# lszmer/metaquest-3d-reconstruction

Hardware: AMD Instinct MI355X
Metric: depth frames/sec integrated + mesh-extract ms, 512³ @ 5 mm; HBM GB/s vs peak (higher is better)
Workload: dtype f32

## Files before the change

### metaquest-3d-reconstruction_amd/csrc/meshfilter.hip

```cpp
#include <hipcub/hipcub.hpp>

#include <algorithm>
#include <cmath>
#include <limits>
#include <map>
#include <mutex>
#include <unordered_map>
#include <vector>

#include "device_block.hpp"
#include "mqr_common.hpp"

namespace mqr {
namespace mf {

__global__ void k_iota(int32_t* a, int64_t n) {
    const int64_t i = (int64_t)blockIdx.x * blockDim.x + threadIdx.x;
    if (i < n) a[i] = (int32_t)i;
}

__global__ void k_edge_keys(const int32_t* __restrict__ tri, int64_t nt, uint64_t* keys, int32_t* slot) {
    const int64_t i = (int64_t)blockIdx.x * blockDim.x + threadIdx.x;
    if (i >= 3 * nt) return;
    const int64_t t = i / 3;
    const int k = (int)(i % 3);
    const uint32_t a = (uint32_t)tri[3 * t + k], b = (uint32_t)tri[3 * t + (k + 1) % 3];
    keys[i] = a < b ? ((uint64_t)a << 32 | b) : ((uint64_t)b << 32 | a);
    slot[i] = (int32_t)i;
}

__device__ inline int32_t uf_find(int32_t* p, int32_t x) {
    while (true) {
        const int32_t px = p[x];
        if (px == x) return x;
        const int32_t gx = p[px];
        if (gx != px) p[x] = gx;
        x = gx;
    }
}

__global__ void k_union_edges(const uint64_t* __restrict__ keys, const int32_t* __restrict__ slot, int64_t m,
                              int32_t* parent) {
    const int64_t i = (int64_t)blockIdx.x * blockDim.x + threadIdx.x;
    if (i == 0 || i >= m || keys[i] != keys[i - 1]) return;
    int32_t a = slot[i - 1] / 3, b = slot[i] / 3;
    while (true) {
        a = uf_find(parent, a);
        b = uf_find(parent, b);
        if (a == b) return;
        if (a > b) {
            const int32_t t = a;
            a = b;
            b = t;
        }
        if (atomicCAS(&parent[b], b, a) == b) return;
    }
}

__global__ void k_roots(int32_t* parent, int64_t n, int32_t* count, int32_t* is_root) {
    const int64_t i = (int64_t)blockIdx.x * blockDim.x + threadIdx.x;
    const int lane = threadIdx.x & 63;
    int32_t r = -1;
    if (i < n) {
        r = uf_find(parent, (int32_t)i);
        is_root[i] = r == (int32_t)i;
    }
    bool todo = i < n;
    while (true) {
        const uint64_t pending = __ballot(todo);
        if (!pending) break;
        const int leader = __ffsll((unsigned long long)pending) - 1;
        const int32_t lr = __shfl(r, leader, 64);
        const bool same = todo && r == lr;
        const uint64_t peers = __ballot(same);
        if (lane == leader) atomicAdd(&count[lr], __popcll(peers));
        if (same) todo = false;
    }
}

__global__ void k_final_root(const int32_t* __restrict__ parent, int64_t n, int32_t* root) {
    const int64_t i = (int64_t)blockIdx.x * blockDim.x + threadIdx.x;
    if (i >= n) return;
    int32_t x = (int32_t)i;
    while (parent[x] != x) x = parent[x];
    root[i] = x;
}

__global__ void k_cluster_table(const int32_t* __restrict__ is_root, const int32_t* __restrict__ cid,
                                const int32_t* __restrict__ count, int64_t n, int32_t* ccount) {
    const int64_t i = (int64_t)blockIdx.x * blockDim.x + threadIdx.x;
    if (i < n && is_root[i]) ccount[cid[i]] = count[i];
}

__global__ void k_keep_by_cluster(const int32_t* __restrict__ root, const int32_t* __restrict__ cid,
                                  const uint8_t* __restrict__ keep_cluster, int64_t n, uint8_t* keep) {
    const int64_t i = (int64_t)blockIdx.x * blockDim.x + threadIdx.x;
    if (i < n) keep[i] = keep_cluster[cid[root[i]]];
}

__global__ void k_gather_tris(const int32_t* __restrict__ tri, const int32_t* __restrict__ sel, int64_t m,
                              int32_t* out) {
    const int64_t i = (int64_t)blockIdx.x * blockDim.x + threadIdx.x;
    if (i >= m) return;
    const int64_t s = sel[i];
    out[3 * i] = tri[3 * s];
    out[3 * i + 1] = tri[3 * s + 1];
    out[3 * i + 2] = tri[3 * s + 2];
}

__global__ void k_mark_vertices(const int32_t* __restrict__ tri, int64_t nt, int32_t* used) {
    const int64_t i = (int64_t)blockIdx.x * blockDim.x + threadIdx.x;
    if (i < 3 * nt) used[tri[i]] = 1;
}

__global__ void k_remap(int32_t* tri, int64_t nt, const int32_t* __restrict__ map) {
    const int64_t i = (int64_t)blockIdx.x * blockDim.x + threadIdx.x;
    if (i < 3 * nt) tri[i] = map[tri[i]];
}

__global__ void k_gather_vertices(const float* __restrict__ pos, const float* __restrict__ nrm,
                                  const int32_t* __restrict__ sel, int64_t m, float* pos_out, float* nrm_out) {
    const int64_t i = (int64_t)blockIdx.x * blockDim.x + threadIdx.x;
    if (i >= m) return;
    const int64_t s = sel[i];
    for (int a = 0; a < 3; ++a) {
        pos_out[3 * i + a] = pos[3 * s + a];
        if (nrm) nrm_out[3 * i + a] = nrm[3 * s + a];
    }
}

__global__ void k_not_degenerate(const int32_t* __restrict__ tri, int64_t nt, uint8_t* keep) {
    const int64_t i = (int64_t)blockIdx.x * blockDim.x + threadIdx.x;
    if (i >= nt) return;
    const int32_t a = tri[3 * i], b = tri[3 * i + 1], c = tri[3 * i + 2];
    keep[i] = a != b && b != c && c != a;
}

__device__ inline void canon(const int32_t* t, uint32_t& k0, uint32_t& k1, uint32_t& k2) {
    const uint32_t a = (uint32_t)t[0], b = (uint32_t)t[1], c = (uint32_t)t[2];
    if (a <= b) {
        if (a <= c) k0 = a, k1 = b, k2 = c;
        else k0 = c, k1 = a, k2 = b;
    } else {
        if (b <= c) k0 = b, k1 = c, k2 = a;
        else k0 = c, k1 = a, k2 = b;
    }
}

__global__ void k_tri_key_lo(const int32_t* __restrict__ tri, int64_t nt, uint32_t* k2, int32_t* idx) {
    const int64_t i = (int64_t)blockIdx.x * blockDim.x + threadIdx.x;
    if (i >= nt) return;
    uint32_t a, b, c;
    canon(tri + 3 * i, a, b, c);
    k2[i] = c;
    idx[i] = (int32_t)i;
}

__global__ void k_tri_key_hi(const int32_t* __restrict__ tri, const int32_t* __restrict__ idx, int64_t nt,
                             uint64_t* k01) {
    const int64_t i = (int64_t)blockIdx.x * blockDim.x + threadIdx.x;
    if (i >= nt) return;
    uint32_t a, b, c;
    canon(tri + 3 * (int64_t)idx[i], a, b, c);
    k01[i] = (uint64_t)a << 32 | b;
}

__global__ void k_first_of_run_tri(const int32_t* __restrict__ tri, const int32_t* __restrict__ idx, int64_t nt,
                                   uint8_t* keep) {
    const int64_t i = (int64_t)blockIdx.x * blockDim.x + threadIdx.x;
    if (i >= nt) return;
    uint32_t a, b, c;
    canon(tri + 3 * (int64_t)idx[i], a, b, c);
    bool first = i == 0;
    if (!first) {
        uint32_t pa, pb, pc;
        canon(tri + 3 * (int64_t)idx[i - 1], pa, pb, pc);
        first = a != pa || b != pb || c != pc;
    }
    keep[idx[i]] = first;
}

__device__ inline uint32_t coord_bits(float f) {
    const uint32_t u = __float_as_uint(f);
    return (u & 0x7fffffffu) == 0 ? 0u : u;
}
__device__ inline bool has_nan(const float* p) { return p[0] != p[0] || p[1] != p[1] || p[2] != p[2]; }

__global__ void k_vtx_key_lo(const float* __restrict__ pos, int64_t nv, uint32_t* kz, int32_t* idx) {
    const int64_t i = (int64_t)blockIdx.x * blockDim.x + threadIdx.x;
    if (i >= nv) return;
    kz[i] = coord_bits(pos[3 * i + 2]);
    idx[i] = (int32_t)i;
}

__global__ void k_vtx_key_hi(const float* __restrict__ pos, const int32_t* __restrict__ idx, int64_t nv,
                             uint64_t* kxy) {
    const int64_t i = (int64_t)blockIdx.x * blockDim.x + threadIdx.x;
    if (i >= nv) return;
    const float* p = pos + 3 * (int64_t)idx[i];
    kxy[i] = (uint64_t)coord_bits(p[0]) << 32 | coord_bits(p[1]);
}

__global__ void k_vtx_heads(const float* __restrict__ pos, const int32_t* __restrict__ idx, int64_t nv,
                            int32_t* head) {
    const int64_t i = (int64_t)blockIdx.x * blockDim.x + threadIdx.x;
    if (i >= nv) return;
    const float* p = pos + 3 * (int64_t)idx[i];
    bool first = i == 0 || has_nan(p);
    if (!first) {
        const float* q = pos + 3 * (int64_t)idx[i - 1];
        first = has_nan(q) || coord_bits(p[0]) != coord_bits(q[0]) || coord_bits(p[1]) != coord_bits(q[1]) ||
                coord_bits(p[2]) != coord_bits(q[2]);
    }
    head[i] = first ? (int32_t)i : 0;
}

__global__ void k_vtx_rep(const int32_t* __restrict__ idx, const int32_t* __restrict__ start, int64_t nv,
                          int32_t* rep, int32_t* keepv) {
    const int64_t i = (int64_t)blockIdx.x * blockDim.x + threadIdx.x;
    if (i >= nv) return;
    const int32_t v = idx[i], r = idx[start[i]];
    rep[v] = r;
    keepv[v] = r == v;
}

__global__ void k_vtx_map(const int32_t* __restrict__ rep, const int32_t* __restrict__ newidx, int64_t nv,
                          int32_t* map) {
    const int64_t i = (int64_t)blockIdx.x * blockDim.x + threadIdx.x;
    if (i < nv) map[i] = newidx[rep[i]];
}

__global__ void k_areas(const float* __restrict__ pos, const int32_t* __restrict__ tri, int64_t nt, double* area) {
    const int64_t i = (int64_t)blockIdx.x * blockDim.x + threadIdx.x;
    if (i >= nt) return;
    const float* p0 = pos + 3 * (int64_t)tri[3 * i];
    const float* p1 = pos + 3 * (int64_t)tri[3 * i + 1];
    const float* p2 = pos + 3 * (int64_t)tri[3 * i + 2];
    const double x0 = (double)p0[0] - p1[0], x1 = (double)p0[1] - p1[1], x2 = (double)p0[2] - p1[2];
    const double y0 = (double)p0[0] - p2[0], y1 = (double)p0[1] - p2[1], y2 = (double)p0[2] - p2[2];
    const double c0 = x1 * y2 - x2 * y1, c1 = x2 * y0 - x0 * y2, c2 = x0 * y1 - x1 * y0;
    area[i] = 0.5 * sqrt((c0 * c0 + c1 * c1) + c2 * c2);
}

__global__ void k_nonmanifold_members(const uint64_t* __restrict__ keys, int64_t m, uint8_t* flag) {
    const int64_t i = (int64_t)blockIdx.x * blockDim.x + threadIdx.x;
    if (i >= m) return;
    const uint64_t k = keys[i];
    const bool p1 = i >= 1 && keys[i - 1] == k, p2 = i >= 2 && keys[i - 2] == k;
    const bool n1 = i + 1 < m && keys[i + 1] == k, n2 = i + 2 < m && keys[i + 2] == k;
    flag[i] = (p1 && p2) || (p1 && n1) || (n1 && n2);
}

__global__ void k_gather_members(const uint64_t* __restrict__ keys, const int32_t* __restrict__ slot,
                                 const double* __restrict__ area, const int32_t* __restrict__ mem, int64_t n,
                                 uint64_t* okey, int32_t* otri, double* oarea) {
    const int64_t i = (int64_t)blockIdx.x * blockDim.x + threadIdx.x;
    if (i >= n) return;
    const int32_t e = mem[i], t = slot[e] / 3;
    okey[i] = keys[e];
    otri[i] = t;
    oarea[i] = area[t];
}

__global__ void k_drop_tris(const int32_t* __restrict__ del, int64_t n, double* area) {
    const int64_t i = (int64_t)blockIdx.x * blockDim.x + threadIdx.x;
    if (i < n) area[del[i]] = -1.0;
}

__global__ void k_keep_positive(const double* __restrict__ area, int64_t nt, uint8_t* keep) {
    const int64_t i = (int64_t)blockIdx.x * blockDim.x + threadIdx.x;
    if (i < nt) keep[i] = area[i] > 0;
}

__global__ void k_gather_f64(const double* __restrict__ a, const int32_t* __restrict__ sel, int64_t m, double* out) {
    const int64_t i = (int64_t)blockIdx.x * blockDim.x + threadIdx.x;
    if (i < m) out[i] = a[sel[i]];
}

inline unsigned nb(int64_t n) { return (unsigned)std::max<int64_t>((n + 255) / 256, 1); }

struct Arena {
    GrowBuf buf;
    bool busy = false;
    hipStream_t s = nullptr;
};
static std::mutex g_arena_mu;
static Arena g_arena[kMaxDevices];

struct Ctx {
    hipStream_t s = nullptr;
    int device = 0;
    Arena* ar = nullptr;
    Arena priv;
    size_t top = 0;
    std::vector<std::pair<size_t, size_t>> stack;
    std::vector<void*> owned;

    int open(int dev, size_t want) {
        device = dev;
        {
            std::lock_guard<std::mutex> lk(g_arena_mu);
            if (dev >= 0 && dev < kMaxDevices && !g_arena[dev].busy) {
                ar = &g_arena[dev];
                ar->busy = true;
            }
        }
        if (!ar) ar = &priv;
        if (!ar->s && hipStreamCreateWithFlags(&ar->s, hipStreamNonBlocking) != hipSuccess) return 1;
        s = ar->s;
        return ar->buf.reserve(want, want) != hipSuccess;
    }
    template <class T>
    T* alloc(int64_t n) {
        const size_t bytes = al256(sizeof(T) * (size_t)std::max<int64_t>(n, 1));
        if (ar && top + bytes <= ar->buf.cap) {
            stack.emplace_back(top, bytes);
            void* p = ar->buf.as<char>() + top;
            top += bytes;
            return static_cast<T*>(p);
        }
        void* p = nullptr;
        if (hipMallocAsync(&p, bytes, s) != hipSuccess) return nullptr;
        owned.push_back(p);
        return static_cast<T*>(p);
    }
    void release(void* p) {
        char* base = ar ? ar->buf.as<char>() : nullptr;
        if (ar && p >= (void*)base && p < (void*)(base + ar->buf.cap)) {
            const size_t off = static_cast<char*>(p) - base;
            for (size_t i = stack.size(); i-- > 0;)
                if (stack[i].first == off) {
                    stack.erase(stack.begin() + (std::ptrdiff_t)i);
                    break;
                }
            top = stack.empty() ? 0 : stack.back().first + stack.back().second;
            return;
        }
        auto it = std::find(owned.begin(), owned.end(), p);
        if (it != owned.end()) {
            (void)hipFreeAsync(p, s);
            owned.erase(it);
        }
    }
    ~Ctx() {
        if (!s) return;
        for (void* p : owned) (void)hipFreeAsync(p, s);
        (void)hipStreamSynchronize(s);
        if (ar == &priv) {
            if (priv.buf.p) (void)hipFree(priv.buf.p);
            (void)hipStreamDestroy(priv.s);
        } else if (ar) {
            std::lock_guard<std::mutex> lk(g_arena_mu);
            ar->busy = false;
        }
    }
};

#define MF_ALLOC(var, T, n)                                                      \
    T* var = c.alloc<T>(n);                                                      \
    if (!var) {                                                                  \
        set_error("mesh filter: device allocation failed");                      \
        return 1;                                                                \
    }

template <class F>
static int select_flagged(Ctx& c, const F* flags, int64_t n, int32_t* out, int64_t* count) {
    hipcub::CountingInputIterator<int32_t> it(0);
    int32_t* d_num = c.alloc<int32_t>(1);
    size_t tb = 0;
    MQR_CHECK_HIP(hipcub::DeviceSelect::Flagged(nullptr, tb, it, flags, out, d_num, (int)n, c.s));
    void* tmp = c.alloc<char>((int64_t)tb + 16);
    if (!d_num || !tmp) {
        set_error("mesh filter: device allocation failed");
        return 1;
    }
    MQR_CHECK_HIP(hipcub::DeviceSelect::Flagged(tmp, tb, it, flags, out, d_num, (int)n, c.s));
    int32_t h = 0;
    MQR_CHECK_HIP(hipMemcpyAsync(&h, d_num, sizeof(int32_t), hipMemcpyDeviceToHost, c.s));
    MQR_CHECK_HIP(hipStreamSynchronize(c.s));
    c.release(tmp);
    c.release(d_num);
    *count = h;
    return 0;
}

static int exclusive_sum(Ctx& c, const int32_t* in, int32_t* out, int64_t n) {
    size_t tb = 0;
    MQR_CHECK_HIP(hipcub::DeviceScan::ExclusiveSum(nullptr, tb, in, out, (int)n, c.s));
    void* tmp = c.alloc<char>((int64_t)tb + 16);
    if (!tmp) {
        set_error("mesh filter: device allocation failed");
        return 1;
    }
    MQR_CHECK_HIP(hipcub::DeviceScan::ExclusiveSum(tmp, tb, in, out, (int)n, c.s));
    c.release(tmp);
    return 0;
}

template <class K>
static int sort_pairs(Ctx& c, const K* kin, K* kout, const int32_t* vin, int32_t* vout, int64_t n, int bits) {
    size_t tb = 0;
    MQR_CHECK_HIP(hipcub::DeviceRadixSort::SortPairs(nullptr, tb, kin, kout, vin, vout, (int)n, 0, bits, c.s));
    void* tmp = c.alloc<char>((int64_t)tb + 16);
    if (!tmp) {
        set_error("mesh filter: device allocation failed");
        return 1;
    }
    MQR_CHECK_HIP(hipcub::DeviceRadixSort::SortPairs(tmp, tb, kin, kout, vin, vout, (int)n, 0, bits, c.s));
    c.release(tmp);
    return 0;
}

struct Mesh {
    float* pos = nullptr;
    float* nrm = nullptr;
    int32_t* tri = nullptr;
    int64_t nv = 0, nt = 0;
};

static int keep_triangles(Ctx& c, Mesh& m, const uint8_t* keep) {
    MF_ALLOC(sel, int32_t, m.nt);
    int64_t k = 0;
    if (select_flagged(c, keep, m.nt, sel, &k)) return 1;
    if (k == m.nt) {
        c.release(sel);
        return 0;
    }
    MF_ALLOC(tri2, int32_t, 3 * k);
    if (k) hipLaunchKernelGGL(k_gather_tris, dim3(nb(k)), dim3(256), 0, c.s, m.tri, sel, k, tri2);
    MQR_CHECK_HIP(hipGetLastError());
    c.release(sel);
    c.release(m.tri);
    m.tri = tri2;
    m.nt = k;
    return 0;
}

static int keep_vertices(Ctx& c, Mesh& m, const int32_t* keepv, const int32_t* map) {
    MF_ALLOC(sel, int32_t, m.nv);
    int64_t k = 0;
    if (select_flagged(c, keepv, m.nv, sel, &k)) return 1;
    if (m.nt) hipLaunchKernelGGL(k_remap, dim3(nb(3 * m.nt)), dim3(256), 0, c.s, m.tri, m.nt, map);
    MQR_CHECK_HIP(hipGetLastError());
    if (k != m.nv) {
        MF_ALLOC(pos2, float, 3 * k);
        float* nrm2 = nullptr;
        if (m.nrm) {
            nrm2 = c.alloc<float>(3 * k);
            if (!nrm2) {
                set_error("mesh filter: device allocation failed");
                return 1;
            }
        }
        if (k) hipLaunchKernelGGL(k_gather_vertices, dim3(nb(k)), dim3(256), 0, c.s, m.pos, m.nrm, sel, k, pos2, nrm2);
        MQR_CHECK_HIP(hipGetLastError());
        c.release(m.pos);
        if (m.nrm) c.release(m.nrm);
        m.pos = pos2;
        m.nrm = nrm2;
        m.nv = k;
    }
    c.release(sel);
    return 0;
}

static int remove_unreferenced_vertices(Ctx& c, Mesh& m) {
    MF_ALLOC(used, int32_t, m.nv);
    MF_ALLOC(newidx, int32_t, m.nv);
    MQR_CHECK_HIP(hipMemsetAsync(used, 0, sizeof(int32_t) * m.nv, c.s));
    if (m.nt) hipLaunchKernelGGL(k_mark_vertices, dim3(nb(3 * m.nt)), dim3(256), 0, c.s, m.tri, m.nt, used);
    MQR_CHECK_HIP(hipGetLastError());
    if (exclusive_sum(c, used, newidx, m.nv)) return 1;
    if (keep_vertices(c, m, used, newidx)) return 1;
    c.release(used);
    c.release(newidx);
    return 0;
}

static int remove_duplicated_triangles(Ctx& c, Mesh& m) {
    if (m.nt < 2) return 0;
    const int64_t n = m.nt;
    MF_ALLOC(k2, uint32_t, n);
    MF_ALLOC(k2s, uint32_t, n);
    MF_ALLOC(idx, int32_t, n);
    MF_ALLOC(idx1, int32_t, n);
    MF_ALLOC(k01, uint64_t, n);
    MF_ALLOC(k01s, uint64_t, n);
    MF_ALLOC(idx2, int32_t, n);
    MF_ALLOC(keep, uint8_t, n);
    hipLaunchKernelGGL(k_tri_key_lo, dim3(nb(n)), dim3(256), 0, c.s, m.tri, n, k2, idx);
    MQR_CHECK_HIP(hipGetLastError());
    if (sort_pairs(c, k2, k2s, idx, idx1, n, 32)) return 1;
    hipLaunchKernelGGL(k_tri_key_hi, dim3(nb(n)), dim3(256), 0, c.s, m.tri, idx1, n, k01);
    MQR_CHECK_HIP(hipGetLastError());
    if (sort_pairs(c, k01, k01s, idx1, idx2, n, 64)) return 1;
    hipLaunchKernelGGL(k_first_of_run_tri, dim3(nb(n)), dim3(256), 0, c.s, m.tri, idx2, n, keep);
    MQR_CHECK_HIP(hipGetLastError());
    if (keep_triangles(c, m, keep)) return 1;
    for (void* p : {(void*)k2, (void*)k2s, (void*)idx, (void*)idx1, (void*)k01, (void*)k01s, (void*)idx2, (void*)keep})
        c.release(p);
    return 0;
}

struct MaxOp {
    __device__ __host__ int32_t operator()(int32_t a, int32_t b) const { return a > b ? a : b; }
};

static int remove_duplicated_vertices(Ctx& c, Mesh& m) {
    if (m.nv < 2) return 0;
    const int64_t n = m.nv;
    MF_ALLOC(kz, uint32_t, n);
    MF_ALLOC(kzs, uint32_t, n);
    MF_ALLOC(idx, int32_t, n);
    MF_ALLOC(idx1, int32_t, n);
    MF_ALLOC(kxy, uint64_t, n);
    MF_ALLOC(kxys, uint64_t, n);
    MF_ALLOC(idx2, int32_t, n);
    MF_ALLOC(head, int32_t, n);
    MF_ALLOC(start, int32_t, n);
    MF_ALLOC(rep, int32_t, n);
    MF_ALLOC(keepv, int32_t, n);
    MF_ALLOC(newidx, int32_t, n);
    MF_ALLOC(map, int32_t, n);
    hipLaunchKernelGGL(k_vtx_key_lo, dim3(nb(n)), dim3(256), 0, c.s, m.pos, n, kz, idx);
    MQR_CHECK_HIP(hipGetLastError());
    if (sort_pairs(c, kz, kzs, idx, idx1, n, 32)) return 1;
    hipLaunchKernelGGL(k_vtx_key_hi, dim3(nb(n)), dim3(256), 0, c.s, m.pos, idx1, n, kxy);
    MQR_CHECK_HIP(hipGetLastError());
    if (sort_pairs(c, kxy, kxys, idx1, idx2, n, 64)) return 1;
    hipLaunchKernelGGL(k_vtx_heads, dim3(nb(n)), dim3(256), 0, c.s, m.pos, idx2, n, head);
    MQR_CHECK_HIP(hipGetLastError());
    {
        size_t tb = 0;
        MQR_CHECK_HIP(hipcub::DeviceScan::InclusiveScan(nullptr, tb, head, start, MaxOp(), (int)n, c.s));
        void* tmp = c.alloc<char>((int64_t)tb + 16);
        if (!tmp) {
            set_error("mesh filter: device allocation failed");
            return 1;
        }
        MQR_CHECK_HIP(hipcub::DeviceScan::InclusiveScan(tmp, tb, head, start, MaxOp(), (int)n, c.s));
        MQR_CHECK_HIP(hipStreamSynchronize(c.s));
        c.release(tmp);
    }
    hipLaunchKernelGGL(k_vtx_rep, dim3(nb(n)), dim3(256), 0, c.s, idx2, start, n, rep, keepv);
    MQR_CHECK_HIP(hipGetLastError());
    if (exclusive_sum(c, keepv, newidx, n)) return 1;
    hipLaunchKernelGGL(k_vtx_map, dim3(nb(n)), dim3(256), 0, c.s, rep, newidx, n, map);
    MQR_CHECK_HIP(hipGetLastError());
    if (keep_vertices(c, m, keepv, map)) return 1;
    for (void* p : {(void*)kz, (void*)kzs, (void*)idx, (void*)idx1, (void*)kxy, (void*)kxys, (void*)idx2, (void*)head,
                    (void*)start, (void*)rep, (void*)keepv, (void*)newidx, (void*)map})
        c.release(p);
    return 0;
}

static int remove_non_manifold_edges(Ctx& c, Mesh& m, int64_t* removed) {
    *removed = 0;
    const int64_t nt0 = m.nt;
    for (int round = 0; round < 1000; ++round) {
        const int64_t n = m.nt;
        if (n == 0) break;
        MF_ALLOC(area, double, n);
        hipLaunchKernelGGL(k_areas, dim3(nb(n)), dim3(256), 0, c.s, m.pos, m.tri, n, area);
        MQR_CHECK_HIP(hipGetLastError());
        const int64_t ne = 3 * n;
        MF_ALLOC(keys, uint64_t, ne);
        MF_ALLOC(keys_s, uint64_t, ne);
        MF_ALLOC(slot, int32_t, ne);
        MF_ALLOC(slot_s, int32_t, ne);
        MF_ALLOC(flag, uint8_t, ne);
        MF_ALLOC(mem, int32_t, ne);
        hipLaunchKernelGGL(k_edge_keys, dim3(nb(ne)), dim3(256), 0, c.s, m.tri, n, keys, slot);
        MQR_CHECK_HIP(hipGetLastError());
        if (sort_pairs(c, keys, keys_s, slot, slot_s, ne, 64)) return 1;
        hipLaunchKernelGGL(k_nonmanifold_members, dim3(nb(ne)), dim3(256), 0, c.s, keys_s, ne, flag);
        MQR_CHECK_HIP(hipGetLastError());
        int64_t nm = 0;
        if (select_flagged(c, flag, ne, mem, &nm)) return 1;
        const bool manifold = nm == 0;
        if (!manifold) {
            MF_ALLOC(mkey, uint64_t, nm);
            MF_ALLOC(mtri, int32_t, nm);
            MF_ALLOC(marea, double, nm);
            hipLaunchKernelGGL(k_gather_members, dim3(nb(nm)), dim3(256), 0, c.s, keys_s, slot_s, area, mem, nm, mkey,
                               mtri, marea);
            MQR_CHECK_HIP(hipGetLastError());
            std::vector<uint64_t> hk(nm);
            std::vector<int32_t> ht(nm);
            std::vector<double> ha(nm);
            MQR_CHECK_HIP(hipMemcpyAsync(hk.data(), mkey, sizeof(uint64_t) * nm, hipMemcpyDeviceToHost, c.s));
            MQR_CHECK_HIP(hipMemcpyAsync(ht.data(), mtri, sizeof(int32_t) * nm, hipMemcpyDeviceToHost, c.s));
            MQR_CHECK_HIP(hipMemcpyAsync(ha.data(), marea, sizeof(double) * nm, hipMemcpyDeviceToHost, c.s));
            MQR_CHECK_HIP(hipStreamSynchronize(c.s));
            std::unordered_map<int32_t, double> cur;
            cur.reserve((size_t)nm);
            for (int64_t j = 0; j < nm; ++j) cur.emplace(ht[j], ha[j]);
            std::vector<int32_t> del;
            for (int64_t s0 = 0; s0 < nm;) {
                int64_t e = s0;
                while (e < nm && hk[e] == hk[s0]) ++e;
                int cnt = 0;
                for (int64_t j = s0; j < e; ++j) cnt += cur[ht[j]] > 0;
                for (int to_delete = cnt - 2; to_delete > 0; --to_delete) {
                    int32_t mt = -1;
                    double ma = std::numeric_limits<double>::max();
                    for (int64_t j = s0; j < e; ++j) {
                        const double a = cur[ht[j]];
                        if (a > 0 && a < ma) mt = ht[j], ma = a;
                    }
                    cur[mt] = -1;
                    del.push_back(mt);
                }
                s0 = e;
            }
            if (!del.empty()) {
                MF_ALLOC(ddel, int32_t, (int64_t)del.size());
                MQR_CHECK_HIP(hipMemcpyAsync(ddel, del.data(), sizeof(int32_t) * del.size(),
                                             hipMemcpyHostToDevice, c.s));
                hipLaunchKernelGGL(k_drop_tris, dim3(nb((int64_t)del.size())), dim3(256), 0, c.s, ddel,
                                   (int64_t)del.size(), area);
                MQR_CHECK_HIP(hipGetLastError());
                MQR_CHECK_HIP(hipStreamSynchronize(c.s));
                c.release(ddel);
            }
            c.release(marea);
            c.release(mtri);
            c.release(mkey);
        }
        MF_ALLOC(keep, uint8_t, n);
        hipLaunchKernelGGL(k_keep_positive, dim3(nb(n)), dim3(256), 0, c.s, area, n, keep);
        MQR_CHECK_HIP(hipGetLastError());
        if (keep_triangles(c, m, keep)) return 1;
        for (void* p : {(void*)area, (void*)keys, (void*)keys_s, (void*)slot, (void*)slot_s, (void*)flag, (void*)mem,
                        (void*)keep})
            c.release(p);
        if (manifold) break;
    }
    *removed = nt0 - m.nt;
    return 0;
}

}
}

using namespace mqr;
using namespace mqr::mf;

extern "C" {

int mqr_mesh_filter_components(int device, const float* vertices, const float* normals, int64_t nv,
                               const int32_t* triangles, int64_t nt, int loc, int64_t min_triangle_count,
                               mqr_geom** out, int64_t* stats) {
    MQR_REQUIRE(out && stats && (nv == 0 || vertices) && (nt == 0 || triangles), "null argument");
    MQR_REQUIRE(nv >= 0 && nt >= 0 && nv < ((int64_t)1 << 31) && nt < ((int64_t)1 << 31) / 3, "mesh too large");
    MQR_CHECK_HIP(hipSetDevice(device));
    for (int i = 0; i < 8; ++i) stats[i] = 0;
    stats[0] = nt;
    Ctx c;
    MQR_REQUIRE(c.open(device, (size_t)(128 * nt + 96 * nv) + ((size_t)32 << 20)) == 0,
                "mesh filter: device allocation failed");
    const hipMemcpyKind k = loc == MQR_DEVICE ? hipMemcpyDeviceToDevice : hipMemcpyHostToDevice;
    if (loc == MQR_DEVICE && order_after_caller(device, c.s)) return 2;
    Mesh m;
    m.nv = nv;
    m.nt = nt;
    m.pos = c.alloc<float>(3 * nv);
    m.nrm = normals ? c.alloc<float>(3 * nv) : nullptr;
    m.tri = c.alloc<int32_t>(3 * nt);
    MQR_REQUIRE(m.pos && m.tri && (!normals || m.nrm), "mesh filter: device allocation failed");
    if (loc == MQR_DEVICE) {
        if (nv) MQR_CHECK_HIP(hipMemcpyAsync(m.pos, vertices, sizeof(float) * 3 * nv, k, c.s));
        if (nv && normals) MQR_CHECK_HIP(hipMemcpyAsync(m.nrm, normals, sizeof(float) * 3 * nv, k, c.s));
        if (nt) MQR_CHECK_HIP(hipMemcpyAsync(m.tri, triangles, sizeof(int32_t) * 3 * nt, k, c.s));
    } else if (copy_to_device(device, m.pos, vertices, sizeof(float) * 3 * nv, c.s) ||
               (normals && copy_to_device(device, m.nrm, normals, sizeof(float) * 3 * nv, c.s)) ||
               copy_to_device(device, m.tri, triangles, sizeof(int32_t) * 3 * nt, c.s)) {
        return 1;
    }
    if (nt > 0) {
        const int64_t ne = 3 * nt;
        int32_t* parent = c.alloc<int32_t>(nt);
        uint64_t* keys = c.alloc<uint64_t>(ne);
        uint64_t* keys_s = c.alloc<uint64_t>(ne);
        int32_t* slot = c.alloc<int32_t>(ne);
        int32_t* slot_s = c.alloc<int32_t>(ne);
        int32_t* count = c.alloc<int32_t>(nt);
        int32_t* is_root = c.alloc<int32_t>(nt);
        int32_t* cid = c.alloc<int32_t>(nt);
        MQR_REQUIRE(parent && keys && keys_s && slot && slot_s && count && is_root && cid,
                    "mesh filter: device allocation failed");
        hipLaunchKernelGGL(k_iota, dim3(nb(nt)), dim3(256), 0, c.s, parent, nt);
        hipLaunchKernelGGL(k_edge_keys, dim3(nb(ne)), dim3(256), 0, c.s, m.tri, nt, keys, slot);
        MQR_CHECK_HIP(hipGetLastError());
        if (sort_pairs(c, keys, keys_s, slot, slot_s, ne, 64)) return 1;
        hipLaunchKernelGGL(k_union_edges, dim3(nb(ne)), dim3(256), 0, c.s, keys_s, slot_s, ne, parent);
        MQR_CHECK_HIP(hipMemsetAsync(count, 0, sizeof(int32_t) * nt, c.s));
        hipLaunchKernelGGL(k_roots, dim3(nb(nt)), dim3(256), 0, c.s, parent, nt, count, is_root);
        int32_t* root = c.alloc<int32_t>(nt);
        MQR_REQUIRE(root, "mesh filter: device allocation failed");
        hipLaunchKernelGGL(k_final_root, dim3(nb(nt)), dim3(256), 0, c.s, parent, nt, root);
        MQR_CHECK_HIP(hipGetLastError());
        if (exclusive_sum(c, is_root, cid, nt)) return 1;
        int32_t last_root = 0, last_cid = 0;
        MQR_CHECK_HIP(hipMemcpyAsync(&last_root, is_root + nt - 1, sizeof(int32_t), hipMemcpyDeviceToHost, c.s));
        MQR_CHECK_HIP(hipMemcpyAsync(&last_cid, cid + nt - 1, sizeof(int32_t), hipMemcpyDeviceToHost, c.s));
        MQR_CHECK_HIP(hipStreamSynchronize(c.s));
        const int64_t C = (int64_t)last_root + last_cid;
        int32_t* ccount = c.alloc<int32_t>(C);
        MQR_REQUIRE(ccount, "mesh filter: device allocation failed");
        hipLaunchKernelGGL(k_cluster_table, dim3(nb(nt)), dim3(256), 0, c.s, is_root, cid, count, nt, ccount);
        MQR_CHECK_HIP(hipGetLastError());
        std::vector<int32_t> h_cc(C);
        MQR_CHECK_HIP(hipMemcpyAsync(h_cc.data(), ccount, sizeof(int32_t) * C, hipMemcpyDeviceToHost, c.s));
        MQR_CHECK_HIP(hipStreamSynchronize(c.s));
        std::vector<uint8_t> keepc(C, 0);
        int64_t kept = 0, largest = 0, kept_tris = 0;
        for (int64_t i = 0; i < C; ++i) {
            largest = std::max<int64_t>(largest, h_cc[i]);
            if (h_cc[i] >= min_triangle_count) keepc[i] = 1, ++kept, kept_tris += h_cc[i];
        }
        if (kept == 0) {
            const int64_t arg = std::max_element(h_cc.begin(), h_cc.end()) - h_cc.begin();
            keepc[arg] = 1;
            kept = 1;
            kept_tris = h_cc[arg];
        }
        stats[1] = C;
        stats[2] = kept;
        stats[3] = nt - kept_tris;
        stats[4] = largest;
        if (kept_tris < nt) {
            uint8_t* d_keepc = c.alloc<uint8_t>(C);
            uint8_t* keep = c.alloc<uint8_t>(nt);
            MQR_REQUIRE(d_keepc && keep, "mesh filter: device allocation failed");
            MQR_CHECK_HIP(hipMemcpyAsync(d_keepc, keepc.data(), C, hipMemcpyHostToDevice, c.s));
            hipLaunchKernelGGL(k_keep_by_cluster, dim3(nb(nt)), dim3(256), 0, c.s, root, cid, d_keepc, nt, keep);
            MQR_CHECK_HIP(hipGetLastError());
            if (keep_triangles(c, m, keep)) return 1;
            if (remove_unreferenced_vertices(c, m)) return 1;
            c.release(d_keepc);
            c.release(keep);
        }
        for (void* p : {(void*)parent, (void*)root, (void*)keys, (void*)keys_s, (void*)slot, (void*)slot_s,
                        (void*)count, (void*)is_root, (void*)cid, (void*)ccount})
            c.release(p);
        if (m.nt) {
            uint8_t* keep = c.alloc<uint8_t>(m.nt);
            MQR_REQUIRE(keep, "mesh filter: device allocation failed");
            hipLaunchKernelGGL(k_not_degenerate, dim3(nb(m.nt)), dim3(256), 0, c.s, m.tri, m.nt, keep);
            MQR_CHECK_HIP(hipGetLastError());
            if (keep_triangles(c, m, keep)) return 1;
            c.release(keep);
        }
        if (remove_duplicated_triangles(c, m)) return 1;
        if (remove_duplicated_vertices(c, m)) return 1;
        int64_t nm_removed = 0;
        if (remove_non_manifold_edges(c, m, &nm_removed)) return 1;
        stats[5] = nm_removed;
    }
    stats[6] = m.nt;
    stats[7] = m.nv;
    mqr_geom* g = new mqr_geom();
    g->device = device;
    g->nv = m.nv;
    g->nt = m.nt;
    if (geom_alloc(g, m.nv, m.nt)) {
        delete g;
        set_error("mesh filter: device allocation failed");
        return 1;
    }
    if (m.nv) MQR_CHECK_HIP(hipMemcpyAsync(g->pos, m.pos, sizeof(float) * 3 * m.nv, hipMemcpyDeviceToDevice, c.s));
    if (m.nv && m.nrm)
        MQR_CHECK_HIP(hipMemcpyAsync(g->nrm, m.nrm, sizeof(float) * 3 * m.nv, hipMemcpyDeviceToDevice, c.s));
    else
        MQR_CHECK_HIP(hipMemsetAsync(g->nrm, 0, (char*)g->tri - (char*)g->nrm, c.s));
    if (m.nt) MQR_CHECK_HIP(hipMemcpyAsync(g->tri, m.tri, sizeof(int32_t) * 3 * m.nt, hipMemcpyDeviceToDevice, c.s));
    MQR_CHECK_HIP(hipStreamSynchronize(c.s));
    *out = g;
    return 0;
}

}
```

Before: 219,400.

## Restructure mesh filter to keep cluster stats on device and reuse sorted edges

Cluster counting, the keep decision and the largest-cluster fallback now run on the GPU through a small stats box, replacing the per-cluster host round trips and the host loop. Duplicate triangles are found from runs in the already-sorted edge keys, and the sorted edge list is carried through compaction so later passes skip re-sorting. Compaction uses count kernels and scans instead of select plus host syncs, and edge keys pack indices into just enough bits. This adds code complexity and a fallback sort path for long key runs, and exact equivalence to the old filtering order is a correctness risk.

Result: no change. 219,100 (-0.2%).

```diff
diff --git a/metaquest-3d-reconstruction_amd/csrc/meshfilter.hip b/metaquest-3d-reconstruction_amd/csrc/meshfilter.hip
--- a/metaquest-3d-reconstruction_amd/csrc/meshfilter.hip
+++ b/metaquest-3d-reconstruction_amd/csrc/meshfilter.hip
@@ -19,13 +19,13 @@
     if (i < n) a[i] = (int32_t)i;
 }
 
-__global__ void k_edge_keys(const int32_t* __restrict__ tri, int64_t nt, uint64_t* keys, int32_t* slot) {
+__global__ void k_edge_keys(const int32_t* __restrict__ tri, int64_t nt, int b, uint64_t* keys, int32_t* slot) {
     const int64_t i = (int64_t)blockIdx.x * blockDim.x + threadIdx.x;
     if (i >= 3 * nt) return;
     const int64_t t = i / 3;
     const int k = (int)(i % 3);
-    const uint32_t a = (uint32_t)tri[3 * t + k], b = (uint32_t)tri[3 * t + (k + 1) % 3];
-    keys[i] = a < b ? ((uint64_t)a << 32 | b) : ((uint64_t)b << 32 | a);
+    const uint64_t u = (uint32_t)tri[3 * t + k], v = (uint32_t)tri[3 * t + (k + 1) % 3];
+    keys[i] = u < v ? (u << b | v) : (v << b | u);
     slot[i] = (int32_t)i;
 }
 
@@ -57,15 +57,47 @@
     }
 }
 
-__global__ void k_roots(int32_t* parent, int64_t n, int32_t* count, int32_t* is_root) {
-    const int64_t i = (int64_t)blockIdx.x * blockDim.x + threadIdx.x;
-    const int lane = threadIdx.x & 63;
+__device__ inline unsigned long long wave_sum(unsigned long long v) {
+    for (int o = 32; o; o >>= 1) v += __shfl_xor(v, o, 64);
+    return v;
+}
+__device__ inline unsigned long long wave_max(unsigned long long v) {
+    for (int o = 32; o; o >>= 1) {
+        const unsigned long long w = __shfl_xor(v, o, 64);
+        v = w > v ? w : v;
+    }
+    return v;
+}
+__device__ inline void block_add(unsigned long long v, unsigned long long* dst) {
+    __shared__ unsigned long long part[16];
+    v = wave_sum(v);
+    if ((threadIdx.x & 63) == 0) part[threadIdx.x >> 6] = v;
+    __syncthreads();
+    if (threadIdx.x == 0) {
+        unsigned long long s = 0;
+        for (unsigned w = 0; w < (blockDim.x + 63) >> 6; ++w) s += part[w];
+        if (s) atomicAdd(dst, s);
+    }
+}
+
+constexpr int kWide = 1024;
+__global__ void __launch_bounds__(kWide) k_roots(const int32_t* __restrict__ parent, int64_t n, int32_t* root,
+                                                 int32_t* count) {
+    __shared__ int32_t w_root[kWide / 64], w_cnt[kWide / 64];
+    const int64_t i = (int64_t)blockIdx.x * blockDim.x + threadIdx.x;
+    const int lane = threadIdx.x & 63, w = threadIdx.x >> 6;
     int32_t r = -1;
     if (i < n) {
-        r = uf_find(parent, (int32_t)i);
-        is_root[i] = r == (int32_t)i;
-    }
-    bool todo = i < n;
+        r = (int32_t)i;
+        while (true) {
+            const int32_t p = parent[r];
+            if (p == r) break;
+            r = p;
+        }
+        root[i] = r;
+    }
+    if (lane == 0) w_cnt[w] = 0;
+    bool todo = i < n, first = true;
     while (true) {
         const uint64_t pending = __ballot(todo);
         if (!pending) break;
@@ -73,67 +105,53 @@
         const int32_t lr = __shfl(r, leader, 64);
         const bool same = todo && r == lr;
         const uint64_t peers = __ballot(same);
-        if (lane == leader) atomicAdd(&count[lr], __popcll(peers));
+        if (lane == leader) {
+            if (first) w_root[w] = lr, w_cnt[w] = __popcll(peers);
+            else atomicAdd(&count[lr], __popcll(peers));
+        }
+        first = false;
         if (same) todo = false;
     }
-}
-
-__global__ void k_final_root(const int32_t* __restrict__ parent, int64_t n, int32_t* root) {
-    const int64_t i = (int64_t)blockIdx.x * blockDim.x + threadIdx.x;
-    if (i >= n) return;
-    int32_t x = (int32_t)i;
-    while (parent[x] != x) x = parent[x];
-    root[i] = x;
-}
-
-__global__ void k_cluster_table(const int32_t* __restrict__ is_root, const int32_t* __restrict__ cid,
-                                const int32_t* __restrict__ count, int64_t n, int32_t* ccount) {
-    const int64_t i = (int64_t)blockIdx.x * blockDim.x + threadIdx.x;
-    if (i < n && is_root[i]) ccount[cid[i]] = count[i];
-}
-
-__global__ void k_keep_by_cluster(const int32_t* __restrict__ root, const int32_t* __restrict__ cid,
-                                  const uint8_t* __restrict__ keep_cluster, int64_t n, uint8_t* keep) {
-    const int64_t i = (int64_t)blockIdx.x * blockDim.x + threadIdx.x;
-    if (i < n) keep[i] = keep_cluster[cid[root[i]]];
-}
-
-__global__ void k_gather_tris(const int32_t* __restrict__ tri, const int32_t* __restrict__ sel, int64_t m,
-                              int32_t* out) {
-    const int64_t i = (int64_t)blockIdx.x * blockDim.x + threadIdx.x;
-    if (i >= m) return;
-    const int64_t s = sel[i];
-    out[3 * i] = tri[3 * s];
-    out[3 * i + 1] = tri[3 * s + 1];
-    out[3 * i + 2] = tri[3 * s + 2];
-}
-
-__global__ void k_mark_vertices(const int32_t* __restrict__ tri, int64_t nt, int32_t* used) {
-    const int64_t i = (int64_t)blockIdx.x * blockDim.x + threadIdx.x;
-    if (i < 3 * nt) used[tri[i]] = 1;
-}
-
-__global__ void k_remap(int32_t* tri, int64_t nt, const int32_t* __restrict__ map) {
-    const int64_t i = (int64_t)blockIdx.x * blockDim.x + threadIdx.x;
-    if (i < 3 * nt) tri[i] = map[tri[i]];
-}
-
-__global__ void k_gather_vertices(const float* __restrict__ pos, const float* __restrict__ nrm,
-                                  const int32_t* __restrict__ sel, int64_t m, float* pos_out, float* nrm_out) {
-    const int64_t i = (int64_t)blockIdx.x * blockDim.x + threadIdx.x;
-    if (i >= m) return;
-    const int64_t s = sel[i];
-    for (int a = 0; a < 3; ++a) {
-        pos_out[3 * i + a] = pos[3 * s + a];
-        if (nrm) nrm_out[3 * i + a] = nrm[3 * s + a];
-    }
-}
-
-__global__ void k_not_degenerate(const int32_t* __restrict__ tri, int64_t nt, uint8_t* keep) {
-    const int64_t i = (int64_t)blockIdx.x * blockDim.x + threadIdx.x;
-    if (i >= nt) return;
-    const int32_t a = tri[3 * i], b = tri[3 * i + 1], c = tri[3 * i + 2];
-    keep[i] = a != b && b != c && c != a;
+    __syncthreads();
+    if (threadIdx.x == 0) {
+        const int nw = (int)(blockDim.x >> 6);
+        for (int a = 0; a < nw; ++a) {
+            if (!w_cnt[a]) continue;
+            int32_t c = w_cnt[a];
+            for (int b = a + 1; b < nw; ++b)
+                if (w_cnt[b] && w_root[b] == w_root[a]) c += w_cnt[b], w_cnt[b] = 0;
+            atomicAdd(&count[w_root[a]], c);
+        }
+    }
+}
+
+enum {
+    kBoxClusters = 0,
+    kBoxKept,
+    kBoxKeptTris,
+    kBoxLargest,
+    kBoxKeepCount,
+    kBoxLongRun,
+    kBoxVertices,
+    kBoxCount,
+    kBoxCount2,
+    kBoxSize = 16
+};
+
+__global__ void k_cluster_stats(const int32_t* __restrict__ root, const int32_t* __restrict__ count, int64_t n,
+                                int64_t min_count, unsigned long long* box) {
+    const int64_t i = (int64_t)blockIdx.x * blockDim.x + threadIdx.x;
+    const bool is_root = i < n && root[i] == (int32_t)i;
+    if (!__ballot(is_root)) return;
+    const unsigned long long cnt = is_root ? (unsigned long long)count[i] : 0;
+    const bool pass = is_root && (int64_t)cnt >= min_count;
+    const unsigned long long c = wave_sum(is_root), k = wave_sum(pass), kt = wave_sum(pass ? cnt : 0);
+    const unsigned long long best = wave_max(is_root ? (cnt << 32 | (0xffffffffu - (uint32_t)i)) : 0);
+    if ((threadIdx.x & 63) == 0) {
+        atomicAdd(&box[kBoxClusters], c);
+        if (k) atomicAdd(&box[kBoxKept], k), atomicAdd(&box[kBoxKeptTris], kt);
+        atomicMax(&box[kBoxLargest], best);
+    }
 }
 
 __device__ inline void canon(const int32_t* t, uint32_t& k0, uint32_t& k1, uint32_t& k2) {
@@ -147,6 +165,114 @@
     }
 }
 
+constexpr int kRunCap = 32;
+__global__ void k_dup_from_runs(const uint64_t* __restrict__ keys, const int32_t* __restrict__ slot, int64_t m,
+                                const int32_t* __restrict__ tri, uint8_t* dup, unsigned long long* box) {
+    const int64_t i = (int64_t)blockIdx.x * blockDim.x + threadIdx.x;
+    if (i >= m) return;
+    const uint64_t key = keys[i];
+    if (i >= kRunCap && keys[i - kRunCap] == key) box[kBoxLongRun] = 1;
+    const int32_t s = slot[i];
+    const int64_t t = s / 3;
+    const int32_t a = tri[3 * t], b = tri[3 * t + 1], c = tri[3 * t + 2];
+    if (a == b || b == c || c == a) return;
+    const int rot = (uint32_t)a <= (uint32_t)b ? ((uint32_t)a <= (uint32_t)c ? 0 : 2)
+                                               : ((uint32_t)b <= (uint32_t)c ? 1 : 2);
+    if (s % 3 != rot) return;
+    uint32_t k0, k1, k2;
+    canon(tri + 3 * t, k0, k1, k2);
+    for (int64_t j = i - 1, steps = 0; j >= 0 && steps < kRunCap && keys[j] == key; --j, ++steps) {
+        uint32_t q0, q1, q2;
+        canon(tri + 3 * (int64_t)(slot[j] / 3), q0, q1, q2);
+        if (q0 == k0 && q1 == k1 && q2 == k2) {
+            dup[t] = 1;
+            return;
+        }
+    }
+}
+
+__global__ void __launch_bounds__(kWide) k_keep_flags(const int32_t* __restrict__ tri, const int32_t* __restrict__ root,
+                             const int32_t* __restrict__ count, const uint8_t* __restrict__ dup, int64_t n,
+                             int64_t min_count, unsigned long long* box, uint8_t* keepc, uint8_t* keep,
+                             int32_t* used) {
+    const int64_t i = (int64_t)blockIdx.x * blockDim.x + threadIdx.x;
+    bool k = false;
+    if (i < n) {
+        const int32_t r = root[i];
+        const bool kc = box[kBoxKept] ? (int64_t)count[r] >= min_count
+                                      : (uint32_t)r == 0xffffffffu - (uint32_t)box[kBoxLargest];
+        const int32_t a = tri[3 * i], b = tri[3 * i + 1], c = tri[3 * i + 2];
+        k = kc && a != b && b != c && c != a && !dup[i];
+        keepc[i] = kc;
+        keep[i] = k;
+        if (kc) used[a] = 1, used[b] = 1, used[c] = 1;
+    }
+    block_add(k, &box[kBoxKeepCount]);
+}
+
+__global__ void __launch_bounds__(kWide) k_count_flags(const uint8_t* __restrict__ flag, int64_t n,
+                                                       unsigned long long* out) {
+    const int64_t i = (int64_t)blockIdx.x * blockDim.x + threadIdx.x;
+    block_add(i < n && flag[i], out);
+}
+
+__global__ void k_scan_total(const int32_t* __restrict__ flag, const int32_t* __restrict__ prefix, int64_t n,
+                             unsigned long long* out) {
+    *out = n ? (unsigned long long)(flag[n - 1] + prefix[n - 1]) : 0;
+}
+
+__global__ void k_compact_tris(const int32_t* __restrict__ tri, const uint8_t* __restrict__ keep,
+                               const int32_t* __restrict__ tmap, const int32_t* __restrict__ vmap, int64_t n,
+                               int32_t* out) {
+    const int64_t i = (int64_t)blockIdx.x * blockDim.x + threadIdx.x;
+    if (i >= n || !keep[i]) return;
+    const int64_t o = 3 * (int64_t)tmap[i];
+    for (int a = 0; a < 3; ++a) {
+        const int32_t v = tri[3 * i + a];
+        out[o + a] = vmap ? vmap[v] : v;
+    }
+}
+
+__global__ void k_carry_edges(const uint64_t* __restrict__ keys, const int32_t* __restrict__ slot,
+                              const int32_t* __restrict__ sel, int64_t m, const int32_t* __restrict__ tmap,
+                              const int32_t* __restrict__ vmap, int b, uint64_t* okeys, int32_t* oslot) {
+    const int64_t i = (int64_t)blockIdx.x * blockDim.x + threadIdx.x;
+    if (i >= m) return;
+    const int64_t e = sel[i];
+    const int32_t s = slot[e];
+    oslot[i] = 3 * tmap[s / 3] + s % 3;
+    uint64_t k = keys[e];
+    if (vmap) {
+        const uint64_t lo = k >> b, hi = k & (((uint64_t)1 << b) - 1);
+        k = (uint64_t)(uint32_t)vmap[lo] << b | (uint32_t)vmap[hi];
+    }
+    okeys[i] = k;
+}
+
+__global__ void k_remap(int32_t* tri, int64_t nt, const int32_t* __restrict__ map) {
+    const int64_t i = (int64_t)blockIdx.x * blockDim.x + threadIdx.x;
+    if (i < 3 * nt) tri[i] = map[tri[i]];
+}
+
+__global__ void k_compact_vertices(const float* __restrict__ pos, const float* __restrict__ nrm,
+                                   const int32_t* __restrict__ keepv, const int32_t* __restrict__ newidx, int64_t n,
+                                   float* pos_out, float* nrm_out) {
+    const int64_t i = (int64_t)blockIdx.x * blockDim.x + threadIdx.x;
+    if (i >= n || !keepv[i]) return;
+    const int64_t o = newidx[i];
+    for (int a = 0; a < 3; ++a) {
+        pos_out[3 * o + a] = pos[3 * i + a];
+        if (nrm) nrm_out[3 * o + a] = nrm[3 * i + a];
+    }
+}
+
+__global__ void k_not_degenerate(const int32_t* __restrict__ tri, int64_t nt, uint8_t* keep) {
+    const int64_t i = (int64_t)blockIdx.x * blockDim.x + threadIdx.x;
+    if (i >= nt) return;
+    const int32_t a = tri[3 * i], b = tri[3 * i + 1], c = tri[3 * i + 2];
+    keep[i] = a != b && b != c && c != a;
+}
+
 __global__ void k_tri_key_lo(const int32_t* __restrict__ tri, int64_t nt, uint32_t* k2, int32_t* idx) {
     const int64_t i = (int64_t)blockIdx.x * blockDim.x + threadIdx.x;
     if (i >= nt) return;
@@ -267,17 +393,16 @@
     if (i < n) area[del[i]] = -1.0;
 }
 
-__global__ void k_keep_positive(const double* __restrict__ area, int64_t nt, uint8_t* keep) {
-    const int64_t i = (int64_t)blockIdx.x * blockDim.x + threadIdx.x;
-    if (i < nt) keep[i] = area[i] > 0;
-}
-
-__global__ void k_gather_f64(const double* __restrict__ a, const int32_t* __restrict__ sel, int64_t m, double* out) {
-    const int64_t i = (int64_t)blockIdx.x * blockDim.x + threadIdx.x;
-    if (i < m) out[i] = a[sel[i]];
+__global__ void __launch_bounds__(kWide) k_keep_positive(const double* __restrict__ area, int64_t nt, uint8_t* keep,
+                                unsigned long long* count) {
+    const int64_t i = (int64_t)blockIdx.x * blockDim.x + threadIdx.x;
+    const bool k = i < nt && area[i] > 0;
+    if (i < nt) keep[i] = k;
+    block_add(k, count);
 }
 
 inline unsigned nb(int64_t n) { return (unsigned)std::max<int64_t>((n + 255) / 256, 1); }
+inline unsigned nbw(int64_t n) { return (unsigned)std::max<int64_t>((n + kWide - 1) / kWide, 1); }
 
 struct Arena {
     GrowBuf buf;
@@ -363,28 +488,23 @@
         return 1;                                                                \
     }
 
-template <class F>
-static int select_flagged(Ctx& c, const F* flags, int64_t n, int32_t* out, int64_t* count) {
+template <class FlagIt>
+static int select_flagged(Ctx& c, FlagIt flags, int64_t n, int32_t* out, int32_t* d_num) {
     hipcub::CountingInputIterator<int32_t> it(0);
-    int32_t* d_num = c.alloc<int32_t>(1);
     size_t tb = 0;
     MQR_CHECK_HIP(hipcub::DeviceSelect::Flagged(nullptr, tb, it, flags, out, d_num, (int)n, c.s));
     void* tmp = c.alloc<char>((int64_t)tb + 16);
-    if (!d_num || !tmp) {
+    if (!tmp) {
         set_error("mesh filter: device allocation failed");
         return 1;
     }
     MQR_CHECK_HIP(hipcub::DeviceSelect::Flagged(tmp, tb, it, flags, out, d_num, (int)n, c.s));
-    int32_t h = 0;
-    MQR_CHECK_HIP(hipMemcpyAsync(&h, d_num, sizeof(int32_t), hipMemcpyDeviceToHost, c.s));
-    MQR_CHECK_HIP(hipStreamSynchronize(c.s));
     c.release(tmp);
-    c.release(d_num);
-    *count = h;
-    return 0;
-}
-
-static int exclusive_sum(Ctx& c, const int32_t* in, int32_t* out, int64_t n) {
+    return 0;
+}
+
+template <class InIt>
+static int exclusive_sum(Ctx& c, InIt in, int32_t* out, int64_t n) {
     size_t tb = 0;
     MQR_CHECK_HIP(hipcub::DeviceScan::ExclusiveSum(nullptr, tb, in, out, (int)n, c.s));
     void* tmp = c.alloc<char>((int64_t)tb + 16);
@@ -411,74 +531,121 @@
     return 0;
 }
 
+struct ToInt {
+    __host__ __device__ int32_t operator()(uint8_t f) const { return f; }
+};
+using FlagInts = hipcub::TransformInputIterator<int32_t, ToInt, const uint8_t*>;
+
+struct EntryKept {
+    const uint8_t* keep;
+    __host__ __device__ uint8_t operator()(int32_t slot) const { return keep[slot / 3]; }
+};
+using EntryFlags = hipcub::TransformInputIterator<uint8_t, EntryKept, const int32_t*>;
+
+static int read_box(Ctx& c, const unsigned long long* box, int first, int n, unsigned long long* h) {
+    MQR_CHECK_HIP(hipMemcpyAsync(h, box + first, sizeof(unsigned long long) * n, hipMemcpyDeviceToHost, c.s));
+    MQR_CHECK_HIP(hipStreamSynchronize(c.s));
+    return 0;
+}
+
+static int count_flags(Ctx& c, const uint8_t* flag, int64_t n, unsigned long long* box, int64_t* count) {
+    MQR_CHECK_HIP(hipMemsetAsync(box + kBoxCount, 0, sizeof(unsigned long long), c.s));
+    hipLaunchKernelGGL(k_count_flags, dim3(nbw(n)), dim3(kWide), 0, c.s, flag, n, box + kBoxCount);
+    MQR_CHECK_HIP(hipGetLastError());
+    unsigned long long h = 0;
+    if (read_box(c, box, kBoxCount, 1, &h)) return 1;
+    *count = (int64_t)h;
+    return 0;
+}
+
 struct Mesh {
     float* pos = nullptr;
     float* nrm = nullptr;
     int32_t* tri = nullptr;
+    int32_t* tri2 = nullptr;
     int64_t nv = 0, nt = 0;
 };
 
-static int keep_triangles(Ctx& c, Mesh& m, const uint8_t* keep) {
-    MF_ALLOC(sel, int32_t, m.nt);
-    int64_t k = 0;
-    if (select_flagged(c, keep, m.nt, sel, &k)) return 1;
-    if (k == m.nt) {
+struct Edges {
+    uint64_t *key = nullptr, *key2 = nullptr;
+    int32_t *slot = nullptr, *slot2 = nullptr;
+    int64_t n = 0;
+    int b = 1;
+    bool valid = false;
+};
+
+static int build_edges(Ctx& c, const Mesh& m, Edges& el) {
+    el.n = 3 * m.nt;
+    hipLaunchKernelGGL(k_edge_keys, dim3(nb(el.n)), dim3(256), 0, c.s, m.tri, m.nt, el.b, el.key, el.slot);
+    MQR_CHECK_HIP(hipGetLastError());
+    hipcub::DoubleBuffer<uint64_t> dk(el.key, el.key2);
+    hipcub::DoubleBuffer<int32_t> dv(el.slot, el.slot2);
+    size_t tb = 0;
+    MQR_CHECK_HIP(hipcub::DeviceRadixSort::SortPairs(nullptr, tb, dk, dv, (int)el.n, 0, 2 * el.b, c.s));
+    void* tmp = c.alloc<char>((int64_t)tb + 16);
+    if (!tmp) {
+        set_error("mesh filter: device allocation failed");
+        return 1;
+    }
+    MQR_CHECK_HIP(hipcub::DeviceRadixSort::SortPairs(tmp, tb, dk, dv, (int)el.n, 0, 2 * el.b, c.s));
+    c.release(tmp);
+    el.key = dk.Current();
+    el.key2 = dk.Alternate();
+    el.slot = dv.Current();
+    el.slot2 = dv.Alternate();
+    el.valid = true;
+    return 0;
+}
+
+static int apply_keep(Ctx& c, Mesh& m, Edges& el, const uint8_t* keep, int64_t k, const int32_t* vmap) {
+    const int64_t n = m.nt;
+    if (k == n && !vmap) return 0;
+    MF_ALLOC(tmap, int32_t, n);
+    if (exclusive_sum(c, FlagInts(keep, ToInt()), tmap, n)) return 1;
+    hipLaunchKernelGGL(k_compact_tris, dim3(nb(n)), dim3(256), 0, c.s, m.tri, keep, tmap, vmap, n, m.tri2);
+    MQR_CHECK_HIP(hipGetLastError());
+    if (el.valid && k) {
+        MF_ALLOC(sel, int32_t, el.n);
+        MF_ALLOC(num, int32_t, 1);
+        if (select_flagged(c, EntryFlags(el.slot, EntryKept{keep}), el.n, sel, num)) return 1;
+        hipLaunchKernelGGL(k_carry_edges, dim3(nb(3 * k)), dim3(256), 0, c.s, el.key, el.slot, sel, 3 * k, tmap, vmap,
+                           el.b, el.key2, el.slot2);
+        MQR_CHECK_HIP(hipGetLastError());
+        std::swap(el.key, el.key2);
+        std::swap(el.slot, el.slot2);
+        c.release(num);
         c.release(sel);
-        return 0;
-    }
-    MF_ALLOC(tri2, int32_t, 3 * k);
-    if (k) hipLaunchKernelGGL(k_gather_tris, dim3(nb(k)), dim3(256), 0, c.s, m.tri, sel, k, tri2);
-    MQR_CHECK_HIP(hipGetLastError());
-    c.release(sel);
-    c.release(m.tri);
-    m.tri = tri2;
+    }
+    el.n = 3 * k;
+    c.release(tmap);
+    std::swap(m.tri, m.tri2);
     m.nt = k;
     return 0;
 }
 
-static int keep_vertices(Ctx& c, Mesh& m, const int32_t* keepv, const int32_t* map) {
-    MF_ALLOC(sel, int32_t, m.nv);
-    int64_t k = 0;
-    if (select_flagged(c, keepv, m.nv, sel, &k)) return 1;
-    if (m.nt) hipLaunchKernelGGL(k_remap, dim3(nb(3 * m.nt)), dim3(256), 0, c.s, m.tri, m.nt, map);
-    MQR_CHECK_HIP(hipGetLastError());
-    if (k != m.nv) {
-        MF_ALLOC(pos2, float, 3 * k);
-        float* nrm2 = nullptr;
-        if (m.nrm) {
-            nrm2 = c.alloc<float>(3 * k);
-            if (!nrm2) {
-                set_error("mesh filter: device allocation failed");
-                return 1;
-            }
-        }
-        if (k) hipLaunchKernelGGL(k_gather_vertices, dim3(nb(k)), dim3(256), 0, c.s, m.pos, m.nrm, sel, k, pos2, nrm2);
-        MQR_CHECK_HIP(hipGetLastError());
-        c.release(m.pos);
-        if (m.nrm) c.release(m.nrm);
-        m.pos = pos2;
-        m.nrm = nrm2;
-        m.nv = k;
-    }
-    c.release(sel);
-    return 0;
-}
-
-static int remove_unreferenced_vertices(Ctx& c, Mesh& m) {
-    MF_ALLOC(used, int32_t, m.nv);
-    MF_ALLOC(newidx, int32_t, m.nv);
-    MQR_CHECK_HIP(hipMemsetAsync(used, 0, sizeof(int32_t) * m.nv, c.s));
-    if (m.nt) hipLaunchKernelGGL(k_mark_vertices, dim3(nb(3 * m.nt)), dim3(256), 0, c.s, m.tri, m.nt, used);
-    MQR_CHECK_HIP(hipGetLastError());
-    if (exclusive_sum(c, used, newidx, m.nv)) return 1;
-    if (keep_vertices(c, m, used, newidx)) return 1;
-    c.release(used);
-    c.release(newidx);
-    return 0;
-}
-
-static int remove_duplicated_triangles(Ctx& c, Mesh& m) {
-    if (m.nt < 2) return 0;
+static int compact_vertices(Ctx& c, Mesh& m, const int32_t* keepv, const int32_t* newidx, int64_t k) {
+    if (k == m.nv) return 0;
+    MF_ALLOC(pos2, float, 3 * k);
+    float* nrm2 = nullptr;
+    if (m.nrm) {
+        nrm2 = c.alloc<float>(3 * k);
+        if (!nrm2) {
+            set_error("mesh filter: device allocation failed");
+            return 1;
+        }
+    }
+    hipLaunchKernelGGL(k_compact_vertices, dim3(nb(m.nv)), dim3(256), 0, c.s, m.pos, m.nrm, keepv, newidx, m.nv, pos2,
+                       nrm2);
+    MQR_CHECK_HIP(hipGetLastError());
+    c.release(m.pos);
+    if (m.nrm) c.release(m.nrm);
+    m.pos = pos2;
+    m.nrm = nrm2;
+    m.nv = k;
+    return 0;
+}
+
+static int first_of_class_by_sort(Ctx& c, const Mesh& m, uint8_t* keep) {
     const int64_t n = m.nt;
     MF_ALLOC(k2, uint32_t, n);
     MF_ALLOC(k2s, uint32_t, n);
@@ -487,7 +654,6 @@
     MF_ALLOC(k01, uint64_t, n);
     MF_ALLOC(k01s, uint64_t, n);
     MF_ALLOC(idx2, int32_t, n);
-    MF_ALLOC(keep, uint8_t, n);
     hipLaunchKernelGGL(k_tri_key_lo, dim3(nb(n)), dim3(256), 0, c.s, m.tri, n, k2, idx);
     MQR_CHECK_HIP(hipGetLastError());
     if (sort_pairs(c, k2, k2s, idx, idx1, n, 32)) return 1;
@@ -496,9 +662,24 @@
     if (sort_pairs(c, k01, k01s, idx1, idx2, n, 64)) return 1;
     hipLaunchKernelGGL(k_first_of_run_tri, dim3(nb(n)), dim3(256), 0, c.s, m.tri, idx2, n, keep);
     MQR_CHECK_HIP(hipGetLastError());
-    if (keep_triangles(c, m, keep)) return 1;
-    for (void* p : {(void*)k2, (void*)k2s, (void*)idx, (void*)idx1, (void*)k01, (void*)k01s, (void*)idx2, (void*)keep})
-        c.release(p);
+    for (void* p : {(void*)k2, (void*)k2s, (void*)idx, (void*)idx1, (void*)k01, (void*)k01s, (void*)idx2}) c.release(p);
+    return 0;
+}
+
+static int remove_degenerate_and_duplicated_by_sort(Ctx& c, Mesh& m, Edges& el, unsigned long long* box) {
+    for (int step = 0; step < 2 && m.nt > step; ++step) {
+        MF_ALLOC(keep, uint8_t, m.nt);
+        if (step == 0) {
+            hipLaunchKernelGGL(k_not_degenerate, dim3(nb(m.nt)), dim3(256), 0, c.s, m.tri, m.nt, keep);
+            MQR_CHECK_HIP(hipGetLastError());
+        } else if (first_of_class_by_sort(c, m, keep)) {
+            return 1;
+        }
+        int64_t k = 0;
+        if (count_flags(c, keep, m.nt, box, &k)) return 1;
+        if (apply_keep(c, m, el, keep, k, nullptr)) return 1;
+        c.release(keep);
+    }
     return 0;
 }
 
@@ -506,7 +687,7 @@
     __device__ __host__ int32_t operator()(int32_t a, int32_t b) const { return a > b ? a : b; }
 };
 
-static int remove_duplicated_vertices(Ctx& c, Mesh& m) {
+static int remove_duplicated_vertices(Ctx& c, Mesh& m, Edges& el, unsigned long long* box) {
     if (m.nv < 2) return 0;
     const int64_t n = m.nv;
     MF_ALLOC(kz, uint32_t, n);
@@ -521,7 +702,6 @@
     MF_ALLOC(rep, int32_t, n);
     MF_ALLOC(keepv, int32_t, n);
     MF_ALLOC(newidx, int32_t, n);
-    MF_ALLOC(map, int32_t, n);
     hipLaunchKernelGGL(k_vtx_key_lo, dim3(nb(n)), dim3(256), 0, c.s, m.pos, n, kz, idx);
     MQR_CHECK_HIP(hipGetLastError());
     if (sort_pairs(c, kz, kzs, idx, idx1, n, 32)) return 1;
@@ -539,50 +719,58 @@
             return 1;
         }
         MQR_CHECK_HIP(hipcub::DeviceScan::InclusiveScan(tmp, tb, head, start, MaxOp(), (int)n, c.s));
-        MQR_CHECK_HIP(hipStreamSynchronize(c.s));
         c.release(tmp);
     }
     hipLaunchKernelGGL(k_vtx_rep, dim3(nb(n)), dim3(256), 0, c.s, idx2, start, n, rep, keepv);
     MQR_CHECK_HIP(hipGetLastError());
-    if (exclusive_sum(c, keepv, newidx, n)) return 1;
-    hipLaunchKernelGGL(k_vtx_map, dim3(nb(n)), dim3(256), 0, c.s, rep, newidx, n, map);
-    MQR_CHECK_HIP(hipGetLastError());
-    if (keep_vertices(c, m, keepv, map)) return 1;
+    if (exclusive_sum(c, (const int32_t*)keepv, newidx, n)) return 1;
+    hipLaunchKernelGGL(k_scan_total, dim3(1), dim3(1), 0, c.s, keepv, newidx, n, box + kBoxCount);
+    MQR_CHECK_HIP(hipGetLastError());
+    unsigned long long k = 0;
+    if (read_box(c, box, kBoxCount, 1, &k)) return 1;
+    if ((int64_t)k != n) {
+        MF_ALLOC(map, int32_t, n);
+        hipLaunchKernelGGL(k_vtx_map, dim3(nb(n)), dim3(256), 0, c.s, rep, newidx, n, map);
+        if (m.nt) hipLaunchKernelGGL(k_remap, dim3(nb(3 * m.nt)), dim3(256), 0, c.s, m.tri, m.nt, map);
+        MQR_CHECK_HIP(hipGetLastError());
+        if (compact_vertices(c, m, keepv, newidx, (int64_t)k)) return 1;
+        c.release(map);
+        el.valid = false;
+    }
     for (void* p : {(void*)kz, (void*)kzs, (void*)idx, (void*)idx1, (void*)kxy, (void*)kxys, (void*)idx2, (void*)head,
-                    (void*)start, (void*)rep, (void*)keepv, (void*)newidx, (void*)map})
+                    (void*)start, (void*)rep, (void*)keepv, (void*)newidx})
         c.release(p);
     return 0;
 }
 
-static int remove_non_manifold_edges(Ctx& c, Mesh& m, int64_t* removed) {
+static int remove_non_manifold_edges(Ctx& c, Mesh& m, Edges& el, unsigned long long* box, int64_t* removed) {
     *removed = 0;
     const int64_t nt0 = m.nt;
     for (int round = 0; round < 1000; ++round) {
         const int64_t n = m.nt;
         if (n == 0) break;
+        if (!el.valid && build_edges(c, m, el)) return 1;
+        const int64_t ne = el.n;
+        MF_ALLOC(keep, uint8_t, n);
         MF_ALLOC(area, double, n);
-        hipLaunchKernelGGL(k_areas, dim3(nb(n)), dim3(256), 0, c.s, m.pos, m.tri, n, area);
-        MQR_CHECK_HIP(hipGetLastError());
-        const int64_t ne = 3 * n;
-        MF_ALLOC(keys, uint64_t, ne);
-        MF_ALLOC(keys_s, uint64_t, ne);
-        MF_ALLOC(slot, int32_t, ne);
-        MF_ALLOC(slot_s, int32_t, ne);
         MF_ALLOC(flag, uint8_t, ne);
         MF_ALLOC(mem, int32_t, ne);
-        hipLaunchKernelGGL(k_edge_keys, dim3(nb(ne)), dim3(256), 0, c.s, m.tri, n, keys, slot);
+        MQR_CHECK_HIP(hipMemsetAsync(box + kBoxCount, 0, 2 * sizeof(unsigned long long), c.s));
+        hipLaunchKernelGGL(k_areas, dim3(nb(n)), dim3(256), 0, c.s, m.pos, m.tri, n, area);
+        hipLaunchKernelGGL(k_keep_positive, dim3(nbw(n)), dim3(kWide), 0, c.s, area, n, keep, box + kBoxCount2);
+        hipLaunchKernelGGL(k_nonmanifold_members, dim3(nb(ne)), dim3(256), 0, c.s, el.key, ne, flag);
         MQR_CHECK_HIP(hipGetLastError());
-        if (sort_pairs(c, keys, keys_s, slot, slot_s, ne, 64)) return 1;
-        hipLaunchKernelGGL(k_nonmanifold_members, dim3(nb(ne)), dim3(256), 0, c.s, keys_s, ne, flag);
-        MQR_CHECK_HIP(hipGetLastError());
-        int64_t nm = 0;
-        if (select_flagged(c, flag, ne, mem, &nm)) return 1;
+        if (select_flagged(c, (const uint8_t*)flag, ne, mem, (int32_t*)(box + kBoxCount))) return 1;
+        unsigned long long h[2] = {0, 0};
+        if (read_box(c, box, kBoxCount, 2, h)) return 1;
+        const int64_t nm = (int64_t)(h[0] & 0xffffffffu);
+        int64_t kept = (int64_t)h[1];
         const bool manifold = nm == 0;
         if (!manifold) {
             MF_ALLOC(mkey, uint64_t, nm);
             MF_ALLOC(mtri, int32_t, nm);
             MF_ALLOC(marea, double, nm);
-            hipLaunchKernelGGL(k_gather_members, dim3(nb(nm)), dim3(256), 0, c.s, keys_s, slot_s, area, mem, nm, mkey,
+            hipLaunchKernelGGL(k_gather_members, dim3(nb(nm)), dim3(256), 0, c.s, el.key, el.slot, area, mem, nm, mkey,
                                mtri, marea);
             MQR_CHECK_HIP(hipGetLastError());
             std::vector<uint64_t> hk(nm);
@@ -619,25 +807,31 @@
                                              hipMemcpyHostToDevice, c.s));
                 hipLaunchKernelGGL(k_drop_tris, dim3(nb((int64_t)del.size())), dim3(256), 0, c.s, ddel,
                                    (int64_t)del.size(), area);
+                hipLaunchKernelGGL(k_keep_positive, dim3(nbw(n)), dim3(kWide), 0, c.s, area, n, keep, box + kBoxCount2);
                 MQR_CHECK_HIP(hipGetLastError());
                 MQR_CHECK_HIP(hipStreamSynchronize(c.s));
+                kept -= (int64_t)del.size();
                 c.release(ddel);
             }
             c.release(marea);
             c.release(mtri);
             c.release(mkey);
         }
-        MF_ALLOC(keep, uint8_t, n);
-        hipLaunchKernelGGL(k_keep_positive, dim3(nb(n)), dim3(256), 0, c.s, area, n, keep);
-        MQR_CHECK_HIP(hipGetLastError());
-        if (keep_triangles(c, m, keep)) return 1;
-        for (void* p : {(void*)area, (void*)keys, (void*)keys_s, (void*)slot, (void*)slot_s, (void*)flag, (void*)mem,
-                        (void*)keep})
-            c.release(p);
+        c.release(mem);
+        c.release(flag);
+        c.release(area);
+        if (apply_keep(c, m, el, keep, kept, nullptr)) return 1;
+        c.release(keep);
         if (manifold) break;
     }
     *removed = nt0 - m.nt;
     return 0;
+}
+
+static int index_bits(int64_t nv) {
+    int b = 1;
+    while (b < 31 && ((int64_t)1 << b) < nv) ++b;
+    return b;
 }
 
 }
@@ -667,7 +861,8 @@
     m.pos = c.alloc<float>(3 * nv);
     m.nrm = normals ? c.alloc<float>(3 * nv) : nullptr;
     m.tri = c.alloc<int32_t>(3 * nt);
-    MQR_REQUIRE(m.pos && m.tri && (!normals || m.nrm), "mesh filter: device allocation failed");
+    m.tri2 = c.alloc<int32_t>(3 * nt);
+    MQR_REQUIRE(m.pos && m.tri && m.tri2 && (!normals || m.nrm), "mesh filter: device allocation failed");
     if (loc == MQR_DEVICE) {
         if (nv) MQR_CHECK_HIP(hipMemcpyAsync(m.pos, vertices, sizeof(float) * 3 * nv, k, c.s));
         if (nv && normals) MQR_CHECK_HIP(hipMemcpyAsync(m.nrm, normals, sizeof(float) * 3 * nv, k, c.s));
@@ -679,83 +874,65 @@
     }
     if (nt > 0) {
         const int64_t ne = 3 * nt;
+        unsigned long long* box = c.alloc<unsigned long long>(kBoxSize);
+        Edges el;
+        el.b = index_bits(nv);
+        el.key = c.alloc<uint64_t>(ne);
+        el.key2 = c.alloc<uint64_t>(ne);
+        el.slot = c.alloc<int32_t>(ne);
+        el.slot2 = c.alloc<int32_t>(ne);
+        uint8_t* keepc = c.alloc<uint8_t>(nt);
+        uint8_t* keep = c.alloc<uint8_t>(nt);
+        int32_t* used = c.alloc<int32_t>(nv);
+        int32_t* newidx = c.alloc<int32_t>(nv);
         int32_t* parent = c.alloc<int32_t>(nt);
-        uint64_t* keys = c.alloc<uint64_t>(ne);
-        uint64_t* keys_s = c.alloc<uint64_t>(ne);
-        int32_t* slot = c.alloc<int32_t>(ne);
-        int32_t* slot_s = c.alloc<int32_t>(ne);
+        int32_t* root = c.alloc<int32_t>(nt);
         int32_t* count = c.alloc<int32_t>(nt);
-        int32_t* is_root = c.alloc<int32_t>(nt);
-        int32_t* cid = c.alloc<int32_t>(nt);
-        MQR_REQUIRE(parent && keys && keys_s && slot && slot_s && count && is_root && cid,
+        uint8_t* dup = c.alloc<uint8_t>(nt);
+        MQR_REQUIRE(box && el.key && el.key2 && el.slot && el.slot2 && keepc && keep && used && newidx && parent &&
+                        root && count && dup,
                     "mesh filter: device allocation failed");
+        MQR_CHECK_HIP(hipMemsetAsync(box, 0, sizeof(unsigned long long) * kBoxSize, c.s));
+        if (build_edges(c, m, el)) return 1;
         hipLaunchKernelGGL(k_iota, dim3(nb(nt)), dim3(256), 0, c.s, parent, nt);
-        hipLaunchKernelGGL(k_edge_keys, dim3(nb(ne)), dim3(256), 0, c.s, m.tri, nt, keys, slot);
+        hipLaunchKernelGGL(k_union_edges, dim3(nb(ne)), dim3(256), 0, c.s, el.key, el.slot, ne, parent);
+        MQR_CHECK_HIP(hipMemsetAsync(count, 0, sizeof(int32_t) * nt, c.s));
+        hipLaunchKernelGGL(k_roots, dim3(nbw(nt)), dim3(kWide), 0, c.s, parent, nt, root, count);
+        hipLaunchKernelGGL(k_cluster_stats, dim3(nb(nt)), dim3(256), 0, c.s, root, count, nt, min_triangle_count, box);
+        MQR_CHECK_HIP(hipMemsetAsync(dup, 0, nt, c.s));
+        MQR_CHECK_HIP(hipMemsetAsync(used, 0, sizeof(int32_t) * nv, c.s));
+        hipLaunchKernelGGL(k_dup_from_runs, dim3(nb(ne)), dim3(256), 0, c.s, el.key, el.slot, ne, m.tri, dup, box);
+        hipLaunchKernelGGL(k_keep_flags, dim3(nbw(nt)), dim3(kWide), 0, c.s, m.tri, root, count, dup, nt,
+                           min_triangle_count, box, keepc, keep, used);
         MQR_CHECK_HIP(hipGetLastError());
-        if (sort_pairs(c, keys, keys_s, slot, slot_s, ne, 64)) return 1;
-        hipLaunchKernelGGL(k_union_edges, dim3(nb(ne)), dim3(256), 0, c.s, keys_s, slot_s, ne, parent);
-        MQR_CHECK_HIP(hipMemsetAsync(count, 0, sizeof(int32_t) * nt, c.s));
-        hipLaunchKernelGGL(k_roots, dim3(nb(nt)), dim3(256), 0, c.s, parent, nt, count, is_root);
-        int32_t* root = c.alloc<int32_t>(nt);
-        MQR_REQUIRE(root, "mesh filter: device allocation failed");
-        hipLaunchKernelGGL(k_final_root, dim3(nb(nt)), dim3(256), 0, c.s, parent, nt, root);
+        if (exclusive_sum(c, (const int32_t*)used, newidx, nv)) return 1;
+        hipLaunchKernelGGL(k_scan_total, dim3(1), dim3(1), 0, c.s, used, newidx, nv, box + kBoxVertices);
         MQR_CHECK_HIP(hipGetLastError());
-        if (exclusive_sum(c, is_root, cid, nt)) return 1;
-        int32_t last_root = 0, last_cid = 0;
-        MQR_CHECK_HIP(hipMemcpyAsync(&last_root, is_root + nt - 1, sizeof(int32_t), hipMemcpyDeviceToHost, c.s));
-        MQR_CHECK_HIP(hipMemcpyAsync(&last_cid, cid + nt - 1, sizeof(int32_t), hipMemcpyDeviceToHost, c.s));
-        MQR_CHECK_HIP(hipStreamSynchronize(c.s));
-        const int64_t C = (int64_t)last_root + last_cid;
-        int32_t* ccount = c.alloc<int32_t>(C);
-        MQR_REQUIRE(ccount, "mesh filter: device allocation failed");
-        hipLaunchKernelGGL(k_cluster_table, dim3(nb(nt)), dim3(256), 0, c.s, is_root, cid, count, nt, ccount);
-        MQR_CHECK_HIP(hipGetLastError());
-        std::vector<int32_t> h_cc(C);
-        MQR_CHECK_HIP(hipMemcpyAsync(h_cc.data(), ccount, sizeof(int32_t) * C, hipMemcpyDeviceToHost, c.s));
-        MQR_CHECK_HIP(hipStreamSynchronize(c.s));
-        std::vector<uint8_t> keepc(C, 0);
-        int64_t kept = 0, largest = 0, kept_tris = 0;
-        for (int64_t i = 0; i < C; ++i) {
-            largest = std::max<int64_t>(largest, h_cc[i]);
-            if (h_cc[i] >= min_triangle_count) keepc[i] = 1, ++kept, kept_tris += h_cc[i];
-        }
-        if (kept == 0) {
-            const int64_t arg = std::max_element(h_cc.begin(), h_cc.end()) - h_cc.begin();
-            keepc[arg] = 1;
-            kept = 1;
-            kept_tris = h_cc[arg];
-        }
-        stats[1] = C;
-        stats[2] = kept;
+        unsigned long long h[kBoxVertices + 1];
+        if (read_box(c, box, 0, kBoxVertices + 1, h)) return 1;
+        const int64_t largest = (int64_t)(h[kBoxLargest] >> 32);
+        const bool none = h[kBoxKept] == 0;
+        const int64_t kept_tris = none ? largest : (int64_t)h[kBoxKeptTris];
+        stats[1] = (int64_t)h[kBoxClusters];
+        stats[2] = none ? 1 : (int64_t)h[kBoxKept];
         stats[3] = nt - kept_tris;
         stats[4] = largest;
-        if (kept_tris < nt) {
-            uint8_t* d_keepc = c.alloc<uint8_t>(C);
-            uint8_t* keep = c.alloc<uint8_t>(nt);
-            MQR_REQUIRE(d_keepc && keep, "mesh filter: device allocation failed");
-            MQR_CHECK_HIP(hipMemcpyAsync(d_keepc, keepc.data(), C, hipMemcpyHostToDevice, c.s));
-            hipLaunchKernelGGL(k_keep_by_cluster, dim3(nb(nt)), dim3(256), 0, c.s, root, cid, d_keepc, nt, keep);
-            MQR_CHECK_HIP(hipGetLastError());
-            if (keep_triangles(c, m, keep)) return 1;
-            if (remove_unreferenced_vertices(c, m)) return 1;
-            c.release(d_keepc);
-            c.release(keep);
-        }
-        for (void* p : {(void*)parent, (void*)root, (void*)keys, (void*)keys_s, (void*)slot, (void*)slot_s,
-                        (void*)count, (void*)is_root, (void*)cid, (void*)ccount})
-            c.release(p);
-        if (m.nt) {
-            uint8_t* keep = c.alloc<uint8_t>(m.nt);
-            MQR_REQUIRE(keep, "mesh filter: device allocation failed");
-            hipLaunchKernelGGL(k_not_degenerate, dim3(nb(m.nt)), dim3(256), 0, c.s, m.tri, m.nt, keep);
-            MQR_CHECK_HIP(hipGetLastError());
-            if (keep_triangles(c, m, keep)) return 1;
-            c.release(keep);
-        }
-        if (remove_duplicated_triangles(c, m)) return 1;
-        if (remove_duplicated_vertices(c, m)) return 1;
+        for (void* p : {(void*)dup, (void*)count, (void*)root, (void*)parent}) c.release(p);
+        const int32_t* vmap = nullptr;
+        if (kept_tris < nt && (int64_t)h[kBoxVertices] < nv) {
+            if (compact_vertices(c, m, used, newidx, (int64_t)h[kBoxVertices])) return 1;
+            vmap = newidx;
+        }
+        if (!h[kBoxLongRun]) {
+            if (apply_keep(c, m, el, keep, (int64_t)h[kBoxKeepCount], vmap)) return 1;
+        } else {
+            if (apply_keep(c, m, el, keepc, kept_tris, vmap)) return 1;
+            if (remove_degenerate_and_duplicated_by_sort(c, m, el, box)) return 1;
+        }
+        for (void* p : {(void*)newidx, (void*)used, (void*)keep, (void*)keepc}) c.release(p);
+        if (remove_duplicated_vertices(c, m, el, box)) return 1;
         int64_t nm_removed = 0;
-        if (remove_non_manifold_edges(c, m, &nm_removed)) return 1;
+        if (remove_non_manifold_edges(c, m, el, box, &nm_removed)) return 1;
         stats[5] = nm_removed;
     }
     stats[6] = m.nt;
```
